# jsh58/Genrich

Hardware: AMD Instinct MI355X
Metric: genome bases p-scored/sec, hg38 50M frags (higher is better)
Workload: dtype int32 pileup (1/120 units) + f64 p-values; 1 GPU; hg38 25 contigs (3088286401 bp), 50000000 paired fragments x 1 replicate(s), treatment only, -p 0.01 (BASELINE.json configs[1]); parallelism=chromosome-sharded x1, collectives=none, rccl_nranks=0, intervals=83948696, tables_written_in_step=none: the sweep walks the loose (end, V) slots, p = table p(V)

## Files before the change

genrich_amd/csrc/gx_stats.h:

```cpp
#pragma once
#include "gx_kernels.h"

namespace gx {


__device__ __forceinline__ float pval_of_v(int v, float lambda, double ml, double sl, float* valOut, bool* neg, bool* risky) {
  float val = getval(v, neg);
  *valOut = val;
  if (lambda == 0.0f) return val == 0.0f ? 0.0f : FLT_MAX;
  return val == 0.0f ? 0.0f : pval_given(val, ml, sl, risky);
}

__device__ __forceinline__ void deep_risky_body(PackIn in, const FragFix* __restrict__ ff, const u32* __restrict__ list,
                                                const Scalars* __restrict__ sc, RiskBuf* __restrict__ risk, u32 block, u32 nBlocks);

__device__ __forceinline__ void lut_entry(u32 v, float lambda, double ml, double sl, float* __restrict__ lutP,
                                          RiskBuf* __restrict__ risk, LooseCtl* __restrict__ ctl, float thr, u32* red, u32 tid,
                                          u32 wg) {
  float val;
  bool ng, risky = false;
  const float p = pval_of_v((int)v, lambda, ml, sl, &val, &ng, &risky);
  lutP[v] = p;
  if (v % GX_UNIT == 0) lutP[PV_LUT + v / GX_UNIT] = p;
  if (risky) risk_add(risk, RK_LUT, v, 0, 0, 0.0);
// ... 893 lines not shown
__global__ __launch_bounds__(QT_NT) void k_qt_apply(const u32* __restrict__ slots, const float* __restrict__ raw, u32 D,
                                                    const float* __restrict__ chunkMin, float* __restrict__ qOfSlot,
                                                    u32* __restrict__ allOne, const u32* __restrict__ Dptr,
                                                    const u64* __restrict__ mins , u32 world, u32 rank) {
  __shared__ float sf[QT_NT / 64 + 4];
  __shared__ float redf[QT_NT / 64];
  __shared__ float preMin;
  if (Dptr) D = *Dptr;
  float before = FLT_MAX;
  if (mins)
    for (u32 o = rank + 1 + threadIdx.x; o < world; o += QT_NT) {
      const float m = __uint_as_float((u32)mins[o]);
      before = m < before ? m : before;
    }
  for (u32 c = threadIdx.x; c < blockIdx.x; c += QT_NT) before = chunkMin[c] < before ? chunkMin[c] : before;
#pragma unroll
  for (int d = 32; d > 0; d >>= 1) {
    const float o = __shfl_xor(before, d, 64);
    before = o < before ? o : before;
  }
  if (lane_id() == 0) redf[threadIdx.x >> 6] = before;
  __syncthreads();
  if (threadIdx.x == 0) {
    float t = FLT_MAX;
    for (int w = 0; w < QT_NT / 64; w++) t = redf[w] < t ? redf[w] : t;
    preMin = t;
  }
  __syncthreads();
  const float chunkBase = preMin;
  const u32 r0 = blockIdx.x * QT_CHUNK + threadIdx.x * QT_ITEMS;
  float rw[QT_ITEMS], mn = FLT_MAX;
#pragma unroll
  for (int k = 0; k < QT_ITEMS; k++) {
    rw[k] = r0 + k < D ? raw[r0 + k] : FLT_MAX;
    mn = rw[k] < mn ? rw[k] : mn;
  }
  float run = block_excl_scan_op<float, QT_NT>(mn, FLT_MAX, sf, OpMinF());
  run = chunkBase < run ? chunkBase : run;
#pragma unroll
  for (int k = 0; k < QT_ITEMS; k++) {
    if (r0 + k < D) {
      run = rw[k] < run ? rw[k] : run;
      const float q = run > 0.0f ? run : 0.0f;
      qOfSlot[slots[D - 1 - (r0 + k)]] = q;
      if (r0 + k == 0 && allOne) *allOne = q == 0.0f;
    }
  }
}

template <int NT, int QL_CACHE_LOG>
__global__ __launch_bounds__(NT) void k_qlookup(const float* __restrict__ p, const u32* __restrict__ nPtr,
                                                const u64* __restrict__ kq, u32 capMask, float* __restrict__ q, float thr, u64* __restrict__ sigMask,
                                                u64* __restrict__ skipMask, u32* __restrict__ st) {
  extern __shared__ __attribute__((aligned(16))) unsigned char ql_raw[];
  u64* lc = reinterpret_cast<u64*>(ql_raw);
  for (int i = threadIdx.x; i < (1 << QL_CACHE_LOG); i += NT) lc[i] = (u64)EMPTY_KEY;
  __syncthreads();
  const u32 n = *nPtr;
  const u32 nw = (n + 63) >> 6;
  constexpr u32 NW = NT / 64;
  for (u32 w0 = (blockIdx.x * NW + (threadIdx.x >> 6)) * 4; w0 < nw; w0 += gridDim.x * NW * 4) {
    float pv[4];
#pragma unroll
    for (int k = 0; k < 4; k++) {
      const u32 i = ((w0 + k) << 6) + lane_id();
      pv[k] = i < n ? p[i] : 0.0f;
    }
#pragma unroll
    for (int k = 0; k < 4; k++) {
      const u32 i = ((w0 + k) << 6) + lane_id();
      float qv = 0.0f;
      if (i < n) {
        if (pv[k] == GX_SKIPF)
          qv = GX_SKIPF;
        else {
          const u32 key = pv[k] == 0.0f ? 0u : __float_as_uint(pv[k]);
          const u32 hh = bh_hash(key);
          const u32 hl = (hh >> 7) & ((1u << QL_CACHE_LOG) - 1);
          const u64 c = lc[hl];
          if ((u32)c == key)
            qv = __uint_as_float((u32)(c >> 32));
          else {
            u32 h = hh & capMask;
            u64 ge;
            while ((u32)(ge = kq[h]) != key && (u32)ge != EMPTY_KEY) h = (h + 1) & capMask;
            if ((u32)ge == key) {
              qv = __uint_as_float((u32)(ge >> 32));
              lc[hl] = ge;
            } else
              atomicOr(st, ST_BH_LEN);
          }
        }
        q[i] = qv;
      }
      const u64 sg = __ballot(i < n && qv > thr), sk = __ballot(i < n && qv == GX_SKIPF);
      if (sigMask && lane_id() == 0 && w0 + k < nw) {
        sigMask[w0 + k] = sg;
        skipMask[w0 + k] = sk;
      }
    }
  }
}

constexpr int SW_NT = 256;
constexpr int SW_ITEMS = 8;
constexpr int SW_CHUNK = SW_NT * SW_ITEMS;
constexpr int RC_CHUNK = SW_NT;

__global__ void k_set_misc(u32* __restrict__ misc, u32 nivWord, u32 genomeWord, u64 genome, u32 n) {
  misc[nivWord] = n;
  *reinterpret_cast<u64*>(misc + genomeWord) = genome;
}

struct SweepMasks {
  u64* sig;
  u64* skip;
  u64* brk;
  u32 nWords;
};

__global__ void k_brk_mask(const u32* __restrict__ chromOff, u32 nChrom, u64* __restrict__ brk) {
  for (u32 c = blockIdx.x * blockDim.x + threadIdx.x; c < nChrom; c += gridDim.x * blockDim.x) {
    u32 a = chromOff[c], b = chromOff[c + 1];
    if (b > a) atomicOr(&brk[a >> 6], 1ull << (a & 63));
  }
}

__global__ __launch_bounds__(256) void k_sig_mask(const float* __restrict__ p, const float* __restrict__ q,
                                                  const u32* __restrict__ nPtr, float thr, SweepMasks M) {
  const u32 n = *nPtr;
  const float* pq = q ? q : p;
  const u32 nw = (n + 63) >> 6;
  for (u32 w0 = (blockIdx.x * 4 + (threadIdx.x >> 6)) * 4; w0 < nw; w0 += gridDim.x * 16) {
    float v[4];
#pragma unroll
    for (int k = 0; k < 4; k++) {
      const u32 i = ((w0 + k) << 6) + lane_id();
      v[k] = i < n ? pq[i] : 0.0f;
    }
#pragma unroll
    for (int k = 0; k < 4; k++) {
      const u64 sg = __ballot(v[k] > thr);
      const u64 sk = __ballot(v[k] == GX_SKIPF);
      if (lane_id() == 0 && w0 + k < nw) {
        M.sig[w0 + k] = sg;
        M.skip[w0 + k] = sk;
      }
    }
  }
}

__device__ __forceinline__ void run_bits(const SweepMasks& M, u32 w, u64* starts, u64* ends) {
  const u64 sg = M.sig[w], bk = M.brk[w];
  const u64 prevBit = w ? M.sig[w - 1] >> 63 : 0ull;
  const u64 nextBit = w + 1 < M.nWords ? M.sig[w + 1] & 1ull : 0ull;
  const u64 nextBrk = w + 1 < M.nWords ? M.brk[w + 1] & 1ull : 0ull;
  *starts = sg & (~((sg << 1) | prevBit) | bk);
  *ends = sg & (~((sg >> 1) | (nextBit << 63)) | ((bk >> 1) | (nextBrk << 63)));
}

__device__ __forceinline__ void run_bits_brk(const SweepMasks& M, u32 w, u64 bk, u64 nextBrk, u64* starts, u64* ends) {
  const u64 sg = M.sig[w];
  const u64 prevBit = w ? M.sig[w - 1] >> 63 : 0ull;
  const u64 nextBit = w + 1 < M.nWords ? M.sig[w + 1] & 1ull : 0ull;
  *starts = sg & (~((sg << 1) | prevBit) | bk);
  *ends = sg & (~((sg >> 1) | (nextBit << 63)) | ((bk >> 1) | (nextBrk << 63)));
}

__device__ __forceinline__ bool any_bit(const u64* __restrict__ mask, u32 lo, u32 hi) {
  if (lo >= hi) return false;
  u32 w0 = lo >> 6, w1 = (hi - 1) >> 6;
  for (u32 w = w0; w <= w1; w++) {
    u64 m = mask[w];
    if (w == w0) m &= ~0ull << (lo & 63);
    if (w == w1 && ((hi & 63) != 0)) m &= (1ull << (hi & 63)) - 1;
    if (m) return true;
  }
  return false;
}

__device__ __forceinline__ bool run_is_head(const SweepMasks& M, const u64* __restrict__ skipMask, const u32* __restrict__ end,
                                            const u32* __restrict__ runStart, const u32* __restrict__ runEnd, u32 r,
                                            int maxGap, const u32* __restrict__ chromOff, u32 nChrom) {
  if (r == 0) return true;
  const u32 a = runEnd[r - 1], s = runStart[r];
  if ((M.brk[s >> 6] >> (s & 63)) & 1ull) return true;
  ChromCursor cur;
  cur.seek(chromOff, nChrom, a);
  if (s >= cur.hi) return true;
  const long long gap = (long long)end[s - 1] - (long long)end[a];
  if (gap != 0 && gap > (long long)maxGap) return true;
  if (skipMask && any_bit(skipMask, a + 1, s)) return true;
  return false;
}

#ifndef GX_PK_SHORT
#define GX_PK_SHORT 1024
#endif
constexpr u32 PK_SHORT = GX_PK_SHORT;
#ifndef GX_PK_LOADS
#define GX_PK_LOADS 8
#endif
constexpr int PK_LOADS = GX_PK_LOADS;

__global__ __launch_bounds__(256) void k_cand_hdr(SweepMasks M, const u32* __restrict__ end,
                                                  const u32* __restrict__ runStart, const u32* __restrict__ runEnd,
                                                  const u32* __restrict__ nRuns, const u32* __restrict__ candRun,
                                                  const u32* __restrict__ nCands, uint4* __restrict__ hdr,
                                                  u32* __restrict__ longList, u32* __restrict__ nLong) {
  const u32 R = *nRuns, C = *nCands;
  for (u32 c = blockIdx.x * 256 + threadIdx.x; c < C; c += gridDim.x * 256) {
    const u32 rFirst = candRun[c], rLast = (c + 1 < C ? candRun[c + 1] : R) - 1;
    const u32 i0 = runStart[rFirst], i1 = runEnd[rLast];
    const bool atChromStart = (M.brk[i0 >> 6] >> (i0 & 63)) & 1ull;
    hdr[c] = make_uint4(i0, i1, atChromStart ? 0u : end[i0 - 1], end[i1]);
    if (i1 - i0 >= PK_SHORT) longList[atomicAdd(nLong, 1u)] = c;
  }
}

__device__ __forceinline__ void peak_finish(u32 c, const uint4 h, float auc, u32 summitPos, float sp, float sq,
                                            float minAUC, int minLen, const u32* __restrict__ chromOff, u32 nChrom,
                                            gx_peak* __restrict__ cand, u32* __restrict__ valid) {
  const u32 peakStart = h.z, peakEnd = h.w;
  const bool ok = auc >= minAUC && (long long)peakEnd - (long long)peakStart >= (long long)minLen;
  valid[c] = ok;
  if (ok) {
    ChromCursor cur;
    cur.seek(chromOff, nChrom, h.x);
    gx_peak pk;
    pk.chrom = cur.c;
    pk.start = peakStart;
    pk.end = peakEnd;
    pk.summit = summitPos;
    pk.auc = auc;
    pk.p = sp;
    pk.q = sq;
    cand[c] = pk;
  }
}

struct PeakAcc {
  float auc = 0.0f, summitVal = -1.0f, sp = -1.0f, sq = -1.0f;
  u32 summitPos = 0, summitLen = 0, s = 0, origin = 0;
  __device__ __forceinline__ void step(u32 e, float pv, float qv, bool useQ, float thr) {
    const float pq = useQ ? qv : pv;
    if (pq > thr) {
      auc += (float)(e - s) * (pq - thr);
      const u32 len = e - s;
      if (pq > summitVal) {
        summitVal = pq;
        sp = pv;
        sq = qv;
        summitPos = (u32)(((u64)e + s) / 2 - origin);
        summitLen = len;
      } else if (pq == summitVal && len > summitLen) {
        summitPos = (u32)(((u64)e + s) / 2 - origin);
        summitLen = len;
      }
    }
    s = e;
  }
};

template <int K> __device__ __forceinline__ float row_lane(float v) {
  return __int_as_float(__builtin_amdgcn_update_dpp(0, __float_as_int(v), 0x150 + K, 0xf, 0xf, false));
}
template <int K> struct RowSeqSum {
  static __device__ __forceinline__ float run(float acc, float v) { return RowSeqSum<K - 1>::run(acc, v) + row_lane<K>(v); }
};
template <> struct RowSeqSum<-1> { static __device__ __forceinline__ float run(float acc, float) { return acc; } };
__device__ __forceinline__ float row_max_f(float v) {
  v = fmaxf(v, __int_as_float(__builtin_amdgcn_update_dpp(0, __float_as_int(v), 0x128, 0xf, 0xf, false)));
  v = fmaxf(v, __int_as_float(__builtin_amdgcn_update_dpp(0, __float_as_int(v), 0x124, 0xf, 0xf, false)));
  v = fmaxf(v, __int_as_float(__builtin_amdgcn_update_dpp(0, __float_as_int(v), 0x122, 0xf, 0xf, false)));
  v = fmaxf(v, __int_as_float(__builtin_amdgcn_update_dpp(0, __float_as_int(v), 0x121, 0xf, 0xf, false)));
  return v;
}
__device__ __forceinline__ u32 row_max_u(u32 v) {
  v = max(v, (u32)__builtin_amdgcn_update_dpp(0, (int)v, 0x128, 0xf, 0xf, false));
  v = max(v, (u32)__builtin_amdgcn_update_dpp(0, (int)v, 0x124, 0xf, 0xf, false));
  v = max(v, (u32)__builtin_amdgcn_update_dpp(0, (int)v, 0x122, 0xf, 0xf, false));
  v = max(v, (u32)__builtin_amdgcn_update_dpp(0, (int)v, 0x121, 0xf, 0xf, false));
  return v;
}

constexpr int PK_AHEAD = 4;
#ifndef GX_PK_AHEAD_V
#define GX_PK_AHEAD_V 4
#endif
__device__ __forceinline__ void load_whole_lut(float* __restrict__ hot, const float* __restrict__ lut) {
  for (u32 i = threadIdx.x; i < PV_WHOLE; i += blockDim.x) hot[i] = lut[PV_LUT + i];
  __syncthreads();
}
__device__ __forceinline__ float p_from_v(const float* __restrict__ hot, const float* __restrict__ lut, const int* __restrict__ V, u32 i) {
  const u32 v = (u32)V[i];
  const u32 c = __umulhi(v, 0x88888889u) >> 6;
  if (v != c * (u32)GX_UNIT) return lut[v < PV_LUT ? v : 0u];
  return hot[c < PV_WHOLE ? c : 0u];
}
__device__ __forceinline__ float q_from_v(const float* __restrict__ hotq, const int* __restrict__ V, u32 i) {
  const u32 c = __umulhi((u32)V[i], 0x88888889u) >> 6;
  return hotq[c < PV_WHOLE ? c : 0u];
}
template <bool USEQ, bool PV, bool PVQ = false>
__device__ __forceinline__ void peak_short_body(const u32 blk, const u32 nBlk, const float* __restrict__ hot, const float* __restrict__ hotq,
                                                const uint4* __restrict__ hdr, const u32* __restrict__ end,
                                                const float* __restrict__ p, const float* __restrict__ q,
                                                const u32* __restrict__ chromOff, u32 nChrom,
                                                const u32* __restrict__ nCands, float thr, float minAUC, int minLen,
                                                gx_peak* __restrict__ cand, u32* __restrict__ valid) {
  constexpr int AH = PV ? GX_PK_AHEAD_V : PK_AHEAD;
  const u32 C = *nCands;
  const int lane = lane_id(), rowBase = lane & 48, rl = lane & 15;
  const u32 rowId = (blk * 4 + (threadIdx.x >> 6)) * 4 + (u32)(lane >> 4);
  for (u32 c0 = 0; c0 < C; c0 += nBlk * 16) {
    const u32 c = c0 + rowId;
    uint4 h = make_uint4(1u, 0u, 0u, 0u);
    if (c < C) h = hdr[c];
    const u32 i0 = h.x, i1 = h.y, peakStart = h.z;
    const bool mine = c < C && i1 - i0 < PK_SHORT;
    const u32 n = mine ? i1 - i0 + 1 : 0u;
    u32 steps = (n + 15) >> 4;
    steps = max(steps, (u32)__shfl_xor((int)steps, 16, 64));
    steps = max(steps, (u32)__shfl_xor((int)steps, 32, 64));
    float auc = 0.0f, summitVal = -1.0f, sp = -1.0f, sq = -1.0f;
    u32 summitPos = 0, summitLen = 0;
    for (u32 st0 = 0; st0 < steps; st0 += AH) {
      u32 e[AH], sPrev[AH];
      float pv[AH], qv[AH];
      bool in[AH];
#pragma unroll
      for (int a = 0; a < AH; a++) {
        const u32 i = i0 + (st0 + a) * 16 + rl;
        in[a] = mine && i <= i1;
        e[a] = 0; sPrev[a] = 0; pv[a] = 0.0f; qv[a] = GX_SKIPF;
        if (in[a]) {
          e[a] = end[i];
          sPrev[a] = i == i0 ? peakStart : end[i - 1];
          if (PV) pv[a] = p_from_v(hot, p, reinterpret_cast<const int*>(q), i);
          else pv[a] = p[i];
          if (USEQ) qv[a] = q[i];
          if (PVQ) qv[a] = q_from_v(hotq, reinterpret_cast<const int*>(q), i);
        }
      }
#pragma unroll
      for (int a = 0; a < AH; a++) {
        if (st0 + a >= steps) break;
        float pq = USEQ || PVQ ? qv[a] : pv[a];
        const bool sg = in[a] && pq > thr;
        float term = 0.0f;
        if (sg) term = (float)(e[a] - sPrev[a]) * (pq - thr);
        else pq = -2.0f;
        const u64 wSg = __ballot(sg);
        if (wSg) {
          auc = RowSeqSum<15>::run(auc, term);
          const float mx = row_max_f(pq);
          const bool atMax = sg && pq == mx;
          const u32 len = atMax ? e[a] - sPrev[a] : 0u;
          const u32 ml = row_max_u(len);
          const bool rowSg = ((u32)(wSg >> rowBase) & 0xFFFFu) != 0;
          const bool better = rowSg && mx > summitVal, longer = rowSg && mx == summitVal && ml > summitLen;
          if (__ballot(better || longer)) {
            const u32 rowMax = (u32)(__ballot(atMax) >> rowBase) & 0xFFFFu;
            const u32 rowLen = (u32)(__ballot(atMax && len == ml) >> rowBase) & 0xFFFFu;
            const int firstMax = rowBase + (rowMax ? __builtin_ctz(rowMax) : 0);
            const int firstLen = rowBase + (rowLen ? __builtin_ctz(rowLen) : 0);
            const u32 myPos = (u32)(((u64)e[a] + sPrev[a]) / 2 - peakStart);
            const u32 cPos = (u32)__shfl((int)myPos, firstLen, 64);
            const float spN = __shfl(pv[a], firstMax, 64), sqN = __shfl(qv[a], firstMax, 64);
            if (better) {
              summitVal = mx;
              sp = spN;
              sq = sqN;
              summitPos = cPos;
              summitLen = ml;
            } else if (longer) {
              summitPos = cPos;
              summitLen = ml;
            }
          }
        }
      }
    }
    if (mine && rl == 0) peak_finish(c, h, auc, summitPos, sp, sq, minAUC, minLen, chromOff, nChrom, cand, valid);
  }
}

template <bool PV, bool PVQ = false>
__device__ __forceinline__ void peak_walk_body(const u32 blk, const u32 nBlk, const float* __restrict__ hot, const float* __restrict__ hotq,
                                               const uint4* __restrict__ hdr, const u32* __restrict__ end,
                                               const float* __restrict__ p, const float* __restrict__ qIn,
                                               const u32* __restrict__ chromOff, u32 nChrom,
                                               const u32* __restrict__ longList, const u32* __restrict__ nLong,
                                               float thr, float minAUC, int minLen,
                                               gx_peak* __restrict__ cand, u32* __restrict__ valid) {
  constexpr int AH = PV ? GX_PK_AHEAD_V : PK_AHEAD;
  const float* __restrict__ q = PV ? nullptr : qIn;
  const u32 L = *nLong;
  const u32 wavesPerGrid = nBlk * 4;
  const int lane = lane_id();
  auto rdf = [](float v, int l) -> float { return __int_as_float(__builtin_amdgcn_readlane(__float_as_int(v), l)); };
  for (u32 li = blk * 4 + (threadIdx.x >> 6); li < L; li += wavesPerGrid) {
    const u32 c = longList[li];
    const uint4 h = hdr[c];
    const u32 i0 = h.x, i1 = h.y, peakStart = h.z;
    float auc = 0.0f, summitVal = -1.0f, sp = -1.0f, sq = -1.0f;
    u32 summitPos = 0, summitLen = 0;
    for (u32 base = i0; base <= i1; base += 64 * AH) {
      u32 e[AH], sPrev[AH];
      float pv[AH], qv[AH];
      bool in[AH];
#pragma unroll
      for (int a = 0; a < AH; a++) {
        const u32 i = base + a * 64 + lane;
        in[a] = i <= i1;
        e[a] = 0; sPrev[a] = 0; pv[a] = 0.0f; qv[a] = GX_SKIPF;
        if (in[a]) {
          e[a] = end[i];
          sPrev[a] = i == i0 ? peakStart : end[i - 1];
          if (PV) pv[a] = p_from_v(hot, p, reinterpret_cast<const int*>(qIn), i);
          else pv[a] = p[i];
          if (q) qv[a] = q[i];
          if (PVQ) qv[a] = q_from_v(hotq, reinterpret_cast<const int*>(qIn), i);
        }
      }
#pragma unroll
      for (int a = 0; a < AH; a++) {
        if (base + a * 64 > i1) break;
        float pq = q || PVQ ? qv[a] : pv[a];
        const bool sg = in[a] && pq > thr;
        float term = 0.0f;
        if (sg) term = (float)(e[a] - sPrev[a]) * (pq - thr);
        else pq = -2.0f;
        if (__ballot(sg)) {
          float acc = RowSeqSum<15>::run(auc, term);
          acc = RowSeqSum<15>::run(rdf(acc, 0), term);
          acc = RowSeqSum<15>::run(rdf(acc, 16), term);
          acc = RowSeqSum<15>::run(rdf(acc, 32), term);
          auc = rdf(acc, 48);
          float mx = row_max_f(pq);
          mx = fmaxf(fmaxf(rdf(mx, 0), rdf(mx, 16)), fmaxf(rdf(mx, 32), rdf(mx, 48)));
          const bool atMax = sg && pq == mx;
          const u32 len = atMax ? e[a] - sPrev[a] : 0u;
          u32 ml = row_max_u(len);
          ml = max(max((u32)__builtin_amdgcn_readlane((int)ml, 0), (u32)__builtin_amdgcn_readlane((int)ml, 16)),
                   max((u32)__builtin_amdgcn_readlane((int)ml, 32), (u32)__builtin_amdgcn_readlane((int)ml, 48)));
          if (mx > summitVal || (mx == summitVal && ml > summitLen)) {
            const int firstMax = __builtin_ctzll(__ballot(atMax));
            const int firstLen = __builtin_ctzll(__ballot(atMax && len == ml));
            const u32 myPos = (u32)(((u64)e[a] + sPrev[a]) / 2 - peakStart);
            const u32 cPos = (u32)__builtin_amdgcn_readlane((int)myPos, firstLen);
            if (mx > summitVal) {
              summitVal = mx;
              sp = rdf(pv[a], firstMax);
              sq = rdf(qv[a], firstMax);
            }
            summitPos = cPos;
            summitLen = ml;
          }
        }
      }
    }
    if (lane == 0) peak_finish(c, h, auc, summitPos, sp, sq, minAUC, minLen, chromOff, nChrom, cand, valid);
  }
}

template <bool USEQ, bool PV, bool PVQ = false>
__global__ __launch_bounds__(256) void k_peak_both(u32 nShort, const uint4* __restrict__ hdr, const u32* __restrict__ end,
                                                   const float* __restrict__ p, const float* __restrict__ q,
                                                   const u32* __restrict__ chromOff, u32 nChrom,
                                                   const u32* __restrict__ nCands, const u32* __restrict__ longList,
                                                   const u32* __restrict__ nLong, float thr, float minAUC, int minLen,
                                                   gx_peak* __restrict__ cand, u32* __restrict__ valid,
                                                   const float* __restrict__ qLut = nullptr) {
  static_assert(!PVQ || (PV && !USEQ), "q by pileup rides the sweep on the loose slots");
  __shared__ float hot[PV ? PV_WHOLE : 1];
  __shared__ float hotq[PVQ ? PV_WHOLE : 1];
  const u32 nWalk = gridDim.x - nShort;
#ifndef GX_PK_NO_EARLY_EXIT
  if (blockIdx.x < nWalk && blockIdx.x * 4 >= *nLong) return;
#endif
  if (PVQ)
    for (u32 i = threadIdx.x; i < PV_WHOLE; i += blockDim.x) hotq[i] = qLut[i];
  if (PV) load_whole_lut(hot, p);
  if (blockIdx.x >= nWalk)
    peak_short_body<USEQ, PV, PVQ>(blockIdx.x - nWalk, nShort, hot, hotq, hdr, end, p, q, chromOff, nChrom, nCands, thr, minAUC, minLen, cand, valid);
  else
    peak_walk_body<PV, PVQ>(blockIdx.x, nWalk, hot, hotq, hdr, end, p, q, chromOff, nChrom, longList, nLong, thr, minAUC, minLen, cand, valid);
}

constexpr int LBG_SHIFT = 38;
__device__ __forceinline__ u64 lookback_gen(u64* lb, u32 id, u64 aggregate, u32 gen, u32* st) {
  const u64 tag = (u64)(gen & 0xFFFFFFu) << LBG_SHIFT, vmask = (1ull << LBG_SHIFT) - 1;
  u64 excl = 0;
  if (id > 0) {
    if (lane_id() == 0)
      __hip_atomic_store(&lb[id], LB_AGG | tag | (aggregate & vmask), __ATOMIC_RELAXED, __HIP_MEMORY_SCOPE_AGENT);
    int look = (int)id - 1;
    u32 spins = 0;
    bool done = false;
    while (!done) {
      const int idx = look - lane_id();
      u64 v = idx >= 0 ? __hip_atomic_load(&lb[idx], __ATOMIC_RELAXED, __HIP_MEMORY_SCOPE_AGENT) : (LB_INC | tag);
      if (((v >> LBG_SHIFT) & 0xFFFFFFu) != (gen & 0xFFFFFFu)) v = 0;
      const u64 flag = v >> 62;
      const u64 invalidMask = __ballot(flag == 0), incMask = __ballot(flag == 2);
      const int firstInvalid = invalidMask ? __builtin_ctzll(invalidMask) : 64;
      const int firstInc = incMask ? __builtin_ctzll(incMask) : 64;
      if (firstInc < firstInvalid) {
        excl += wave_sum(lane_id() <= firstInc ? (v & vmask) : 0ull);
        done = true;
      } else if (firstInvalid > 0) {
        excl += wave_sum(lane_id() < firstInvalid ? (v & vmask) : 0ull);
        look -= firstInvalid;
      } else {
        __builtin_amdgcn_s_sleep(1);
        ++spins;
        bool abort_ = spins > LB_SPIN_LIMIT;
        if (!abort_ && (spins & 1023u) == 0)
          abort_ = (__hip_atomic_load(st, __ATOMIC_RELAXED, __HIP_MEMORY_SCOPE_AGENT) & ST_LOOKBACK) != 0;
        if (abort_) {
          if (lane_id() == 0) atomicOr(st, ST_LOOKBACK);
          done = true;
        }
      }
    }
  }
  excl &= vmask;
  if (lane_id() == 0)
    __hip_atomic_store(&lb[id], LB_INC | tag | ((excl + aggregate) & vmask), __ATOMIC_RELAXED, __HIP_MEMORY_SCOPE_AGENT);
  return excl;
}

struct ChromStarts {
  const DChrom* chroms = nullptr;
  const u32* tileSlot = nullptr;
  u32 nChrom = 0;
};
constexpr u32 RUN_NCH = 1024;

struct RunsOut {
  u32* runStart;
  u32* runEnd;
  u32 cap;
  u32* nRuns;
  u32* nRunsHost;
  u32* zeroMe;
  u64* zeroBp;
};

template <bool TABLE>
__device__ __forceinline__ void runs_body(const SweepMasks& M, const ChromStarts& CS, u64* __restrict__ lbS, u64* __restrict__ lbE,
                                          u32 gen, const RunsOut& O, u32* __restrict__ st, u32 wg, u32 nWg) {
  u32* __restrict__ runStart = O.runStart;
  u32* __restrict__ runEnd = O.runEnd;
  const u32 cap = O.cap;
  __shared__ u32 scratch[8];
  __shared__ u64 s_base[2];
  __shared__ u64 s_brk[TABLE ? SW_CHUNK + 1 : 1];
  __shared__ u32 s_cstart[TABLE ? RUN_NCH : 1];
  const u32 nChunks = (M.nWords + SW_CHUNK - 1) / SW_CHUNK;
  const bool cached = TABLE && CS.nChrom <= RUN_NCH;
  auto chrom_start = [&](u32 c) {
    const u32 tb = CS.chroms[c].tileBase;
    return tb != NULL_TILE ? CS.tileSlot[tb] : ~0u;
  };
  if (cached && wg < nChunks) {
    for (u32 c = threadIdx.x; c < CS.nChrom; c += SW_NT) s_cstart[c] = chrom_start(c);
  }
  for (u32 id = wg; id < nChunks; id += nWg) {
    const u32 w0 = id * SW_CHUNK + threadIdx.x * SW_ITEMS;
    if (TABLE) {
      for (u32 i = threadIdx.x; i < SW_CHUNK + 1; i += SW_NT) s_brk[i] = 0;
      __syncthreads();
      const u64 lo = (u64)id * SW_CHUNK * 64, hi = lo + (u64)(SW_CHUNK + 1) * 64;
      for (u32 c = threadIdx.x; c < CS.nChrom; c += SW_NT) {
        const u32 a = cached ? s_cstart[c] : chrom_start(c);
        if (a != ~0u && a >= lo && a < hi) atomicOr((unsigned long long*)&s_brk[(a >> 6) - id * SW_CHUNK], 1ull << (a & 63));
      }
      __syncthreads();
    }
    u64 stb[SW_ITEMS], enb[SW_ITEMS];
    u32 a = 0, b = 0;
#pragma unroll
    for (int k = 0; k < SW_ITEMS; k++) {
      stb[k] = 0;
      enb[k] = 0;
      if (w0 + k < M.nWords) {
        if (TABLE) {
          const u32 l = threadIdx.x * SW_ITEMS + k;
          run_bits_brk(M, w0 + k, s_brk[l], w0 + k + 1 < M.nWords ? s_brk[l + 1] & 1ull : 0ull, &stb[k], &enb[k]);
        } else
          run_bits(M, w0 + k, &stb[k], &enb[k]);
      }
      a += __popcll(stb[k]);
      b += __popcll(enb[k]);
    }
    u32 totA;
    u32 oa = block_excl_scan<u32, SW_NT>(a, scratch, &totA);
    (void)b;
    if (threadIdx.x < 64) {
      const u64 ea = lookback_gen(lbS, id, totA, gen, st);
      if (threadIdx.x == 0) {
        s_base[0] = ea;
        if (id == nChunks - 1) {
          const u32 total = (u32)ea + totA;
          *O.nRuns = total > cap ? cap : total;
          *O.nRunsHost = total;
          *O.zeroMe = 0;
          *O.zeroBp = 0;
        }
      }
    }
    __syncthreads();
    oa += (u32)s_base[0];
    u32 ob = oa;
    if (w0 < M.nWords) {
      const u64 sig0 = M.sig[w0];
      ob -= (u32)(sig0 & ~stb[0] & 1ull);
    }
#ifdef GX_RUNS_TWO_SCANS
    {
      u32 totB;
      ob = block_excl_scan<u32, SW_NT>(b, scratch, &totB);
      __shared__ u64 s_b;
      if (threadIdx.x < 64) {
        const u64 eb = lookback_gen(lbE, id, totB, gen, st);
        if (threadIdx.x == 0) s_b = eb;
      }
      __syncthreads();
      ob += (u32)s_b;
    }
#endif
#pragma unroll
    for (int k = 0; k < SW_ITEMS; k++) {
      u64 x = stb[k];
      while (x) {
        const int bit = __builtin_ctzll(x);
        x &= x - 1;
        if (oa < cap) runStart[oa] = ((w0 + k) << 6) + bit;
        oa++;
      }
      x = enb[k];
      while (x) {
        const int bit = __builtin_ctzll(x);
        x &= x - 1;
        if (ob < cap) runEnd[ob] = ((w0 + k) << 6) + bit;
        ob++;
      }
    }
    __syncthreads();
  }
}

template <bool TABLE>
__global__ __launch_bounds__(SW_NT) void k_runs(SweepMasks M, ChromStarts CS, u64* __restrict__ lbS, u64* __restrict__ lbE, u32 gen,
                                                RunsOut O, u32* __restrict__ st) {
  runs_body<TABLE>(M, CS, lbS, lbE, gen, O, st, blockIdx.x, gridDim.x);
}

struct RunHalf {
  SweepMasks M;
  ChromStarts CS;
  u64* lbS;
  u64* lbE;
  u32 gen;
  RunsOut O;
  u32 nScan;
};
__global__ __launch_bounds__(STL_NT) void k_scan_iv_close_runs(const u32* __restrict__ tileCount, const u32* __restrict__ tileLastEnd,
                                                               const u32* __restrict__ tileChrom, const DChrom* __restrict__ chroms,
                                                               u32 nTiles, u64* __restrict__ lbSum, u64* __restrict__ lbMax,
                                                               IvScanOut out, u32* __restrict__ st, CloseArgs C, RunHalf R) {
  static_assert(STL_NT == SW_NT, "one workgroup size for both halves");
  if (blockIdx.x < R.nScan)
    scan_close_body(tileCount, tileLastEnd, tileChrom, chroms, nTiles, lbSum, lbMax, out, st, C, blockIdx.x, R.nScan);
  else
    runs_body<true>(R.M, R.CS, R.lbS, R.lbE, R.gen, R.O, st, blockIdx.x - R.nScan, gridDim.x - R.nScan);
}

__global__ __launch_bounds__(SW_NT) void k_cands(SweepMasks M, const u64* __restrict__ skipMask, const u32* __restrict__ end,
                                                 const u32* __restrict__ runStart, const u32* __restrict__ runEnd,
                                                 const u32* __restrict__ nRuns, int maxGap, const u32* __restrict__ chromOff,
                                                 u32 nChrom, u64* __restrict__ lb, u32 gen, u32* __restrict__ candRun,
                                                 u32* __restrict__ nCands, u32* __restrict__ st) {
  __shared__ u32 scratch[8];
  __shared__ u64 s_base;
  const u32 R = *nRuns;
  const u32 nChunks = (R + RC_CHUNK - 1) / RC_CHUNK;
  if (nChunks == 0 && blockIdx.x == 0 && threadIdx.x == 0) *nCands = 0;
  for (u32 id = blockIdx.x; id < nChunks; id += gridDim.x) {
    const u32 r = id * RC_CHUNK + threadIdx.x;
    const u32 keep = r < R ? (u32)run_is_head(M, skipMask, end, runStart, runEnd, r, maxGap, chromOff, nChrom) : 0u;
    u32 tot;
    u32 o = block_excl_scan<u32, SW_NT>(keep, scratch, &tot);
    if (threadIdx.x < 64) {
      const u64 e = lookback_gen(lb, id, tot, gen, st);
      if (threadIdx.x == 0) {
        s_base = e;
        if (id == nChunks - 1) *nCands = (u32)e + tot;
      }
    }
    __syncthreads();
    if (keep) candRun[o + (u32)s_base] = r;
    __syncthreads();
  }
}

__global__ __launch_bounds__(SW_NT) void k_peaks(const gx_peak* __restrict__ cand, const u32* __restrict__ valid,
                                                 const u32* __restrict__ nHeads, u64* __restrict__ lb, u32 gen,
                                                 gx_peak* __restrict__ peaks , u32* __restrict__ nPeaks,
                                                 u32* __restrict__ nPeaksHost, u32* __restrict__ st,
                                                 u64* __restrict__ bpAcc ) {
  constexpr int PW = sizeof(gx_peak) / 4;
  __shared__ u32 scratch[8];
  __shared__ u32 stage[RC_CHUNK * PW];
  __shared__ u64 s_base;
  const u32 H = *nHeads;
  const u32 nChunks = (H + RC_CHUNK - 1) / RC_CHUNK;
  u64 bp = 0;
  if (nChunks == 0 && blockIdx.x == 0 && threadIdx.x == 0) {
    *nPeaks = 0;
    *nPeaksHost = 0;
  }
  for (u32 id = blockIdx.x; id < nChunks; id += gridDim.x) {
    const u32 h = id * RC_CHUNK + threadIdx.x;
    const u32 keep = h < H ? valid[h] : 0u;
    u32 tot;
    const u32 r = block_excl_scan<u32, SW_NT>(keep, scratch, &tot);
    if (keep) {
      const u32* src = reinterpret_cast<const u32*>(cand + h);
#pragma unroll
      for (int k = 0; k < PW; k++) stage[r * PW + k] = src[k];
      bp += cand[h].end - cand[h].start;
    }
    if (threadIdx.x < 64) {
      const u64 e = lookback_gen(lb, id, tot, gen, st);
      if (threadIdx.x == 0) {
        s_base = e;
        if (id == nChunks - 1) {
          *nPeaks = (u32)e + tot;
          *nPeaksHost = (u32)e + tot;
        }
      }
    }
    __syncthreads();
    u32* dst = reinterpret_cast<u32*>(peaks + (u32)s_base);
    for (u32 i = threadIdx.x; i < tot * PW; i += SW_NT) dst[i] = stage[i];
    __syncthreads();
  }
  __shared__ unsigned long long s_bp;
  if (threadIdx.x == 0) s_bp = 0;
  __syncthreads();
  bp = wave_sum(bp);
  if (lane_id() == 0 && bp) atomicAdd(&s_bp, (unsigned long long)bp);
  __syncthreads();
  if (threadIdx.x == 0 && s_bp) atomicAdd((unsigned long long*)bpAcc, s_bp);
}

}
```

Before: 2907 Gbases/s.

## Process two peak intervals per lane with paired loads and DPP previous-end shuffles

Restructures the short-peak scan so each lane in a 16-lane row handles two consecutive intervals, loading end and value arrays as 64-bit pairs when they are 8-byte aligned. The previous interval's end now comes from a DPP row shift carrying the last lane's value instead of a second global load of end[i-1], and the walk path uses a wave-wide DPP shift the same way. The intent is to halve the per-interval load instructions and remove the redundant neighbour loads, at the cost of extra boundary handling for odd start indices and the last slot, plus a separate narrow fallback instantiation.

New measurement: 2949 Gbases/s (median of 6 runs). +1.5%, better.

```diff
diff --git a/genrich_amd/csrc/gx_stats.h b/genrich_amd/csrc/gx_stats.h
--- a/genrich_amd/csrc/gx_stats.h
+++ b/genrich_amd/csrc/gx_stats.h
@@ -1219,14 +1219,72 @@
   const u32 c = __umulhi((u32)V[i], 0x88888889u) >> 6;
   return hotq[c < PV_WHOLE ? c : 0u];
 }
-template <bool USEQ, bool PV, bool PVQ = false>
+__device__ __forceinline__ float2 p_from_v2(const float* __restrict__ hot, const float* __restrict__ lut, u32 v0, u32 v1) {
+  const u32 c0 = __umulhi(v0, 0x88888889u) >> 6, c1 = __umulhi(v1, 0x88888889u) >> 6;
+  float r0 = hot[c0 < PV_WHOLE ? c0 : 0u], r1 = hot[c1 < PV_WHOLE ? c1 : 0u];
+  const bool f0 = v0 != c0 * (u32)GX_UNIT, f1 = v1 != c1 * (u32)GX_UNIT;
+  if (__ballot(f0 || f1)) {
+    const float t0 = lut[f0 && v0 < PV_LUT ? v0 : 0u], t1 = lut[f1 && v1 < PV_LUT ? v1 : 0u];
+    if (f0) r0 = t0;
+    if (f1) r1 = t1;
+  }
+  return make_float2(r0, r1);
+}
+__device__ __forceinline__ float q_of_v(const float* __restrict__ hotq, u32 v) {
+  const u32 c = __umulhi(v, 0x88888889u) >> 6;
+  return hotq[c < PV_WHOLE ? c : 0u];
+}
+
+template <bool WIDE> __device__ __forceinline__ uint2 pk_ld2(const u32* a) {
+  if (WIDE) return *reinterpret_cast<const uint2*>(a);
+  return make_uint2(a[0], a[1]);
+}
+template <int K> __device__ __forceinline__ u32 row_lane_u(u32 v) {
+  return (u32)__builtin_amdgcn_update_dpp(0, (int)v, 0x150 + K, 0xf, 0xf, false);
+}
+__device__ __forceinline__ u32 row_prev_u(u32 first, u32 v) {
+  return (u32)__builtin_amdgcn_update_dpp((int)first, (int)v, 0x111, 0xf, 0xf, false);
+}
+__device__ __forceinline__ u32 wave_prev_u(u32 first, u32 v) {
+  return (u32)__builtin_amdgcn_update_dpp((int)first, (int)v, 0x138, 0xf, 0xf, false);
+}
+template <int K> struct RowSeqSum2 {
+  static __device__ __forceinline__ float run(float acc, float a, float b) {
+    return (RowSeqSum2<K - 1>::run(acc, a, b) + row_lane<K>(a)) + row_lane<K>(b);
+  }
+};
+template <> struct RowSeqSum2<-1> { static __device__ __forceinline__ float run(float acc, float, float) { return acc; } };
+
+template <int AH, bool USEQ> struct PkGroup {
+  uint2 e[AH], a[AH], b[USEQ ? AH : 1];
+};
+template <bool WIDE, bool USEQ, int AH>
+__device__ __forceinline__ void pk_load(PkGroup<AH, USEQ>& G, const u32* __restrict__ end, const u32* __restrict__ a,
+                                        const u32* __restrict__ b, const u32* __restrict__ spare, u32 idx, u32 i1, bool mine) {
+#pragma unroll
+  for (int k = 0; k < AH; k++, idx += 32) {
+    const bool ok = mine && idx < i1;
+    G.e[k] = pk_ld2<WIDE>(ok ? end + idx : spare);
+    G.a[k] = pk_ld2<WIDE>(ok ? a + idx : spare);
+    if (USEQ) G.b[k] = pk_ld2<WIDE>(ok ? b + idx : spare);
+  }
+}
+
+#ifndef GX_PK_PAIR_STEPS
+#define GX_PK_PAIR_STEPS 2
+#endif
+constexpr int PK_PAIR_STEPS = GX_PK_PAIR_STEPS;
+template <bool WIDE, bool USEQ, bool PV, bool PVQ>
 __device__ __forceinline__ void peak_short_body(const u32 blk, const u32 nBlk, const float* __restrict__ hot, const float* __restrict__ hotq,
                                                 const uint4* __restrict__ hdr, const u32* __restrict__ end,
                                                 const float* __restrict__ p, const float* __restrict__ q,
                                                 const u32* __restrict__ chromOff, u32 nChrom,
                                                 const u32* __restrict__ nCands, float thr, float minAUC, int minLen,
                                                 gx_peak* __restrict__ cand, u32* __restrict__ valid) {
-  constexpr int AH = PV ? GX_PK_AHEAD_V : PK_AHEAD;
+  constexpr int AH = PK_PAIR_STEPS;
+  const u32* __restrict__ arrA = reinterpret_cast<const u32*>(PV ? q : p);
+  const u32* __restrict__ arrB = reinterpret_cast<const u32*>(q);
+  const u32* __restrict__ spare = reinterpret_cast<const u32*>(hdr);
   const u32 C = *nCands;
   const int lane = lane_id(), rowBase = lane & 48, rl = lane & 15;
   const u32 rowId = (blk * 4 + (threadIdx.x >> 6)) * 4 + (u32)(lane >> 4);
@@ -1234,57 +1292,74 @@
     const u32 c = c0 + rowId;
     uint4 h = make_uint4(1u, 0u, 0u, 0u);
     if (c < C) h = hdr[c];
-    const u32 i0 = h.x, i1 = h.y, peakStart = h.z;
+    const u32 i0 = h.x, i1 = h.y, peakStart = h.z, peakEnd = h.w;
     const bool mine = c < C && i1 - i0 < PK_SHORT;
-    const u32 n = mine ? i1 - i0 + 1 : 0u;
-    u32 steps = (n + 15) >> 4;
+    const u32 idxL = (i0 & ~1u) + 2u * (u32)rl;
+    u32 steps = mine ? (i1 - (i0 & ~1u) + 32) >> 5 : 0u;
     steps = max(steps, (u32)__shfl_xor((int)steps, 16, 64));
     steps = max(steps, (u32)__shfl_xor((int)steps, 32, 64));
+    const u32 lastA = *(mine ? arrA + i1 : spare), lastB = USEQ ? *(mine ? arrB + i1 : spare) : 0u;
     float auc = 0.0f, summitVal = -1.0f, sp = -1.0f, sq = -1.0f;
-    u32 summitPos = 0, summitLen = 0;
+    u32 summitPos = 0, summitLen = 0, carry = 0;
     for (u32 st0 = 0; st0 < steps; st0 += AH) {
-      u32 e[AH], sPrev[AH];
-      float pv[AH], qv[AH];
-      bool in[AH];
-#pragma unroll
-      for (int a = 0; a < AH; a++) {
-        const u32 i = i0 + (st0 + a) * 16 + rl;
-        in[a] = mine && i <= i1;
-        e[a] = 0; sPrev[a] = 0; pv[a] = 0.0f; qv[a] = GX_SKIPF;
-        if (in[a]) {
-          e[a] = end[i];
-          sPrev[a] = i == i0 ? peakStart : end[i - 1];
-          if (PV) pv[a] = p_from_v(hot, p, reinterpret_cast<const int*>(q), i);
-          else pv[a] = p[i];
-          if (USEQ) qv[a] = q[i];
-          if (PVQ) qv[a] = q_from_v(hotq, reinterpret_cast<const int*>(q), i);
+      PkGroup<AH, USEQ> cur;
+      pk_load<WIDE, USEQ, AH>(cur, end, arrA, arrB, spare, idxL + 32u * st0, i1, mine);
+#pragma unroll
+      for (int k = 0; k < AH; k++) {
+        if (st0 + k >= steps) break;
+        const u32 idx = idxL + 32u * (st0 + k);
+        uint2 ee = cur.e[k], va = cur.a[k], vb = USEQ ? cur.b[k] : make_uint2(0u, 0u);
+        const bool in0 = mine && idx >= i0 && idx <= i1, in1 = mine && idx < i1;
+        if (idx == i1) {
+          ee.x = peakEnd;
+          va.x = lastA;
+          vb.x = lastB;
         }
-      }
-#pragma unroll
-      for (int a = 0; a < AH; a++) {
-        if (st0 + a >= steps) break;
-        float pq = USEQ || PVQ ? qv[a] : pv[a];
-        const bool sg = in[a] && pq > thr;
-        float term = 0.0f;
-        if (sg) term = (float)(e[a] - sPrev[a]) * (pq - thr);
-        else pq = -2.0f;
-        const u64 wSg = __ballot(sg);
+        float pv0, pv1, qv0 = GX_SKIPF, qv1 = GX_SKIPF;
+        if (PV) {
+          const float2 pp = p_from_v2(hot, p, in0 ? va.x : 0u, in1 ? va.y : 0u);
+          pv0 = pp.x;
+          pv1 = pp.y;
+        } else {
+          pv0 = __uint_as_float(va.x);
+          pv1 = __uint_as_float(va.y);
+        }
+        if (USEQ) {
+          qv0 = __uint_as_float(vb.x);
+          qv1 = __uint_as_float(vb.y);
+        }
+        if (PVQ) {
+          qv0 = q_of_v(hotq, in0 ? va.x : 0u);
+          qv1 = q_of_v(hotq, in1 ? va.y : 0u);
+        }
+        const u32 before = row_prev_u(carry, ee.y);
+        const u32 s0 = idx == i0 ? peakStart : before, s1 = idx + 1 == i0 ? peakStart : ee.x;
+        carry = row_lane_u<15>(ee.y);
+        float pq0 = USEQ || PVQ ? qv0 : pv0, pq1 = USEQ || PVQ ? qv1 : pv1;
+        const bool sg0 = in0 && pq0 > thr, sg1 = in1 && pq1 > thr;
+        float t0 = 0.0f, t1 = 0.0f;
+        if (sg0) t0 = (float)(ee.x - s0) * (pq0 - thr);
+        else pq0 = -2.0f;
+        if (sg1) t1 = (float)(ee.y - s1) * (pq1 - thr);
+        else pq1 = -2.0f;
+        const u64 wSg = __ballot(sg0 || sg1);
         if (wSg) {
-          auc = RowSeqSum<15>::run(auc, term);
-          const float mx = row_max_f(pq);
-          const bool atMax = sg && pq == mx;
-          const u32 len = atMax ? e[a] - sPrev[a] : 0u;
-          const u32 ml = row_max_u(len);
+          auc = RowSeqSum2<15>::run(auc, t0, t1);
+          const float mx = row_max_f(fmaxf(pq0, pq1));
+          const bool am0 = sg0 && pq0 == mx, am1 = sg1 && pq1 == mx;
+          const u32 len0 = am0 ? ee.x - s0 : 0u, len1 = am1 ? ee.y - s1 : 0u;
+          const u32 ml = row_max_u(max(len0, len1));
           const bool rowSg = ((u32)(wSg >> rowBase) & 0xFFFFu) != 0;
           const bool better = rowSg && mx > summitVal, longer = rowSg && mx == summitVal && ml > summitLen;
           if (__ballot(better || longer)) {
-            const u32 rowMax = (u32)(__ballot(atMax) >> rowBase) & 0xFFFFu;
-            const u32 rowLen = (u32)(__ballot(atMax && len == ml) >> rowBase) & 0xFFFFu;
+            const bool l0 = am0 && len0 == ml, l1 = am1 && len1 == ml;
+            const u32 rowMax = (u32)(__ballot(am0 || am1) >> rowBase) & 0xFFFFu;
+            const u32 rowLen = (u32)(__ballot(l0 || l1) >> rowBase) & 0xFFFFu;
             const int firstMax = rowBase + (rowMax ? __builtin_ctz(rowMax) : 0);
             const int firstLen = rowBase + (rowLen ? __builtin_ctz(rowLen) : 0);
-            const u32 myPos = (u32)(((u64)e[a] + sPrev[a]) / 2 - peakStart);
+            const u32 myPos = l0 ? (u32)(((u64)ee.x + s0) / 2 - peakStart) : (u32)(((u64)ee.y + s1) / 2 - peakStart);
             const u32 cPos = (u32)__shfl((int)myPos, firstLen, 64);
-            const float spN = __shfl(pv[a], firstMax, 64), sqN = __shfl(qv[a], firstMax, 64);
+            const float spN = __shfl(am0 ? pv0 : pv1, firstMax, 64), sqN = __shfl(am0 ? qv0 : qv1, firstMax, 64);
             if (better) {
               summitVal = mx;
               sp = spN;
@@ -1302,6 +1377,7 @@
     if (mine && rl == 0) peak_finish(c, h, auc, summitPos, sp, sq, minAUC, minLen, chromOff, nChrom, cand, valid);
   }
 }
+
 
 template <bool PV, bool PVQ = false>
 __device__ __forceinline__ void peak_walk_body(const u32 blk, const u32 nBlk, const float* __restrict__ hot, const float* __restrict__ hotq,
@@ -1322,19 +1398,18 @@
     const uint4 h = hdr[c];
     const u32 i0 = h.x, i1 = h.y, peakStart = h.z;
     float auc = 0.0f, summitVal = -1.0f, sp = -1.0f, sq = -1.0f;
-    u32 summitPos = 0, summitLen = 0;
+    u32 summitPos = 0, summitLen = 0, carry = 0;
     for (u32 base = i0; base <= i1; base += 64 * AH) {
-      u32 e[AH], sPrev[AH];
+      u32 e[AH];
       float pv[AH], qv[AH];
       bool in[AH];
 #pragma unroll
       for (int a = 0; a < AH; a++) {
         const u32 i = base + a * 64 + lane;
         in[a] = i <= i1;
-        e[a] = 0; sPrev[a] = 0; pv[a] = 0.0f; qv[a] = GX_SKIPF;
+        e[a] = 0; pv[a] = 0.0f; qv[a] = GX_SKIPF;
         if (in[a]) {
           e[a] = end[i];
-          sPrev[a] = i == i0 ? peakStart : end[i - 1];
           if (PV) pv[a] = p_from_v(hot, p, reinterpret_cast<const int*>(qIn), i);
           else pv[a] = p[i];
           if (q) qv[a] = q[i];
@@ -1344,10 +1419,13 @@
 #pragma unroll
       for (int a = 0; a < AH; a++) {
         if (base + a * 64 > i1) break;
+        const u32 before = wave_prev_u(carry, e[a]);
+        const u32 sPrev = base + a * 64 + lane == i0 ? peakStart : before;
+        carry = (u32)__builtin_amdgcn_readlane((int)e[a], 63);
         float pq = q || PVQ ? qv[a] : pv[a];
         const bool sg = in[a] && pq > thr;
         float term = 0.0f;
-        if (sg) term = (float)(e[a] - sPrev[a]) * (pq - thr);
+        if (sg) term = (float)(e[a] - sPrev) * (pq - thr);
         else pq = -2.0f;
         if (__ballot(sg)) {
           float acc = RowSeqSum<15>::run(auc, term);
@@ -1358,14 +1436,14 @@
           float mx = row_max_f(pq);
           mx = fmaxf(fmaxf(rdf(mx, 0), rdf(mx, 16)), fmaxf(rdf(mx, 32), rdf(mx, 48)));
           const bool atMax = sg && pq == mx;
-          const u32 len = atMax ? e[a] - sPrev[a] : 0u;
+          const u32 len = atMax ? e[a] - sPrev : 0u;
           u32 ml = row_max_u(len);
           ml = max(max((u32)__builtin_amdgcn_readlane((int)ml, 0), (u32)__builtin_amdgcn_readlane((int)ml, 16)),
                    max((u32)__builtin_amdgcn_readlane((int)ml, 32), (u32)__builtin_amdgcn_readlane((int)ml, 48)));
           if (mx > summitVal || (mx == summitVal && ml > summitLen)) {
             const int firstMax = __builtin_ctzll(__ballot(atMax));
             const int firstLen = __builtin_ctzll(__ballot(atMax && len == ml));
-            const u32 myPos = (u32)(((u64)e[a] + sPrev[a]) / 2 - peakStart);
+            const u32 myPos = (u32)(((u64)e[a] + sPrev) / 2 - peakStart);
             const u32 cPos = (u32)__builtin_amdgcn_readlane((int)myPos, firstLen);
             if (mx > summitVal) {
               summitVal = mx;
@@ -1400,8 +1478,15 @@
   if (PVQ)
     for (u32 i = threadIdx.x; i < PV_WHOLE; i += blockDim.x) hotq[i] = qLut[i];
   if (PV) load_whole_lut(hot, p);
-  if (blockIdx.x >= nWalk)
-    peak_short_body<USEQ, PV, PVQ>(blockIdx.x - nWalk, nShort, hot, hotq, hdr, end, p, q, chromOff, nChrom, nCands, thr, minAUC, minLen, cand, valid);
+#ifdef GX_PK_NARROW
+  const bool wide = false;
+#else
+  const bool wide = (((uintptr_t)end | (uintptr_t)(PV ? nullptr : p) | (uintptr_t)(USEQ || PV ? q : nullptr)) & 7) == 0;
+#endif
+  if (blockIdx.x >= nWalk && wide)
+    peak_short_body<true, USEQ, PV, PVQ>(blockIdx.x - nWalk, nShort, hot, hotq, hdr, end, p, q, chromOff, nChrom, nCands, thr, minAUC, minLen, cand, valid);
+  else if (blockIdx.x >= nWalk)
+    peak_short_body<false, USEQ, PV, PVQ>(blockIdx.x - nWalk, nShort, hot, hotq, hdr, end, p, q, chromOff, nChrom, nCands, thr, minAUC, minLen, cand, valid);
   else
     peak_walk_body<PV, PVQ>(blockIdx.x, nWalk, hot, hotq, hdr, end, p, q, chromOff, nChrom, longList, nLong, thr, minAUC, minLen, cand, valid);
 }
```
